# Canleskis/ephemeris-explorer

Hardware: AMD Instinct MI355X
Metric: body-steps/s (higher is better)
Workload: dtype f64

## Files before the change

### ephemeris_explorer_amd/csrc/step_wg.hip

```cpp
#include <algorithm>
#include <type_traits>
#include <utility>

#include "pair_ns.h"

#ifndef EPH_EXPERIMENTS
#define EPH_EXPERIMENTS 0
#endif
#if !EPH_EXPERIMENTS || !defined(EPH_WG_SIDE)
#undef EPH_WG_SIDE
#define EPH_WG_SIDE 0
#endif
#if !EPH_EXPERIMENTS || !defined(EPH_WG_ABLATE)
#undef EPH_WG_ABLATE
#define EPH_WG_ABLATE 0
#endif
#define WG_LOOP_BARRIER() do { if constexpr (!(EPH_WG_ABLATE & 2)) __syncthreads(); } while (0)
#if EPH_EXPERIMENTS && defined(EPH_WG_DIAG_PATCH)
#define EPH_WG_DIAG_PATCH_ON 1
#else
#define EPH_WG_DIAG_PATCH_ON 0
#endif


namespace eph {
namespace EPH_PV_NS {

constexpr int kWgBodies = 16;
constexpr int kDuoThreads = 64 * 6;
constexpr int kDuoTailWave = 5;
constexpr int kWgChainWave = 4;
constexpr int kWgTailWave = 8;
constexpr int kWgThreads = 64 * 12;
constexpr int kWgTileBufs = 6;
constexpr int kWgSplitBufs = 3;

template <int NB>
__device__ __forceinline__ void wg_pair_tile(const double (&xi)[NB], const double (&yi)[NB], const double (&zi)[NB],
                                             const Body4 &pj, bool ieee, double *tile, int b0, int lane) {
    PairPre pre[NB];
    unsigned worst = ieee ? kRangeSpan : mu_key(pj.mu), low = ~0u;
#pragma unroll
    for (int b = 0; b < NB; ++b) {
        pre[b] = pair_pre(xi[b], yi[b], zi[b], pj);
        worst = max(worst, range_key(pre[b].n2));
        low = min(low, pre[b].lo);
    }
    worst = max(worst, low_key(low));
    double c[3 * NB];
    if (__builtin_amdgcn_ballot_w64(worst >= kRangeSpan) == 0) {
#pragma unroll
        for (int b = 0; b < NB; ++b) pair_finish<true>(pre[b], pj.mu, c[3 * b], c[3 * b + 1], c[3 * b + 2]);
    } else {
#pragma unroll
        for (int b = 0; b < NB; ++b) pair_finish<false>(pre[b], pj.mu, c[3 * b], c[3 * b + 1], c[3 * b + 2]);
    }
#pragma unroll
    for (int q = 0; q < 3 * NB; ++q) {
        if constexpr (EPH_WG_ABLATE & 1) asm volatile("" ::"v"(c[q]));
        else tile[(3 * b0 + q) * kRow + lane] = c[q];
    }
}

template <int NB, typename PosPtr>
__device__ __forceinline__ void wg_pair_wave(PosPtr pos, int n, int i0, int b0, double *C, int lane, int tiles, int tdiag, int wbuf) {
    double xi[NB], yi[NB], zi[NB];
#pragma unroll
    for (int b = 0; b < NB; ++b) {
        const int ii = min(i0 + b0 + b, n - 1);
        xi[b] = pos[ii].x;
        yi[b] = pos[ii].y;
        zi[b] = pos[ii].z;
    }
    auto load_src = [&](int t) -> Body4 {
        const int j = min(t, tiles - 1) * kTile + lane;
        return pos[j < n ? j : n - 1];
    };
    Body4 pj = load_src(0);
    Body4 pjn = load_src(1);
    wg_pair_tile<NB>(xi, yi, zi, pj, tdiag == 0, C, b0, lane);
    pj = pjn;
    pjn = load_src(2);
    if (tiles > 1) wg_pair_tile<NB>(xi, yi, zi, pj, tdiag == 1, C + wbuf, b0, lane);
    __syncthreads();
    for (int t = 0; t < tiles; ++t) {
        if (t + 2 < tiles) {
            pj = pjn;
            pjn = load_src(t + 3);
            wg_pair_tile<NB>(xi, yi, zi, pj, tdiag == t + 2, C + ((t + 2) % kWgSplitBufs) * wbuf, b0, lane);
        }
        __syncthreads();
    }
}

template <int NB>
__device__ __forceinline__ void wg_pair_tile2(const double (&xi)[NB], const double (&yi)[NB], const double (&zi)[NB],
                                              const Body4 &pa, const Body4 &pb, bool ieee, double *tile_a, double *tile_b,
                                              int b0, int lane, int self_a = -64, int self_b = -64) {
    PairPre pre[2 * NB];
    unsigned worst = ieee ? kRangeSpan : max(mu_key(pa.mu), mu_key(pb.mu)), low = ~0u;
#pragma unroll
    for (int b = 0; b < NB; ++b) {
        pre[b] = pair_pre(xi[b], yi[b], zi[b], pa);
        pre[NB + b] = pair_pre(xi[b], yi[b], zi[b], pb);
        if constexpr (EPH_WG_DIAG_PATCH_ON) {
            if (lane == self_a + b) { pre[b].n2 = 1.0; pre[b].lo = 0x3ff00000u; }
            if (lane == self_b + b) { pre[NB + b].n2 = 1.0; pre[NB + b].lo = 0x3ff00000u; }
        }
        worst = max(worst, max(range_key(pre[b].n2), range_key(pre[NB + b].n2)));
        low = min(low, min(pre[b].lo, pre[NB + b].lo));
    }
    worst = max(worst, low_key(low));
    double c[6 * NB];
    if (__builtin_amdgcn_ballot_w64(worst >= kRangeSpan) == 0) {
        if constexpr (kPairStaged) {
            double mus[2 * NB];
#pragma unroll
            for (int b = 0; b < NB; ++b) { mus[b] = pa.mu; mus[NB + b] = pb.mu; }
            pair_finish_staged<2 * NB>(pre, mus, c);
        } else {
#pragma unroll
            for (int b = 0; b < NB; ++b) {
                pair_finish<true>(pre[b], pa.mu, c[3 * b], c[3 * b + 1], c[3 * b + 2]);
                pair_finish<true>(pre[NB + b], pb.mu, c[3 * (NB + b)], c[3 * (NB + b) + 1], c[3 * (NB + b) + 2]);
            }
        }
    } else {
#pragma unroll
        for (int b = 0; b < NB; ++b) {
            pair_finish<false>(pre[b], pa.mu, c[3 * b], c[3 * b + 1], c[3 * b + 2]);
            pair_finish<false>(pre[NB + b], pb.mu, c[3 * (NB + b)], c[3 * (NB + b) + 1], c[3 * (NB + b) + 2]);
        }
    }
#pragma unroll
    for (int q = 0; q < 3 * NB; ++q) {
        if constexpr (EPH_WG_ABLATE & 1) {
            asm volatile("" ::"v"(c[q]), "v"(c[3 * NB + q]));
        } else {
            tile_a[(3 * b0 + q) * kRow + lane] = c[q];
            tile_b[(3 * b0 + q) * kRow + lane] = c[3 * NB + q];
        }
    }
}

__device__ __forceinline__ int big_start(int K) { return K < 2 ? K : 2 * K - 2; }
__device__ __forceinline__ int big_count(int tiles) { return tiles <= 2 ? tiles : 2 + (tiles - 2 + 1) / 2; }
template <int NB, typename PosPtr>
__device__ __forceinline__ void wg_pair_wave_big(PosPtr pos, int n, int i0, int b0, double *C, int lane, int tiles, int tdiag, int wbuf) {
    double xi[NB], yi[NB], zi[NB];
#pragma unroll
    for (int b = 0; b < NB; ++b) {
        const int ii = min(i0 + b0 + b, n - 1);
        xi[b] = pos[ii].x;
        yi[b] = pos[ii].y;
        zi[b] = pos[ii].z;
    }
    auto load_src = [&](int t) -> Body4 {
        const int j = min(t, tiles - 1) * kTile + lane;
        return pos[j < n ? j : n - 1];
    };
    auto produce = [&](int K, const Body4 &pa, const Body4 &pb) {
        const int t = big_start(K);
        if (t >= tiles || EPH_WG_SIDE == 2) return;
        double *ta = C + (t % kWgTileBufs) * wbuf, *tb = C + ((t + 1) % kWgTileBufs) * wbuf;
        if constexpr (EPH_WG_DIAG_PATCH_ON) {
            if (K >= 2 && t + 1 < tiles) {
                const int own = i0 + b0;
                wg_pair_tile2<NB>(xi, yi, zi, pa, pb, false, ta, tb, b0, lane, tdiag == t ? own - t * kTile : -64,
                                  tdiag == t + 1 ? own - (t + 1) * kTile : -64);
                return;
            }
        }
        if (K >= 2 && t + 1 < tiles) wg_pair_tile2<NB>(xi, yi, zi, pa, pb, tdiag == t || tdiag == t + 1, ta, tb, b0, lane);
        else wg_pair_tile<NB>(xi, yi, zi, pa, tdiag == t, ta, b0, lane);
    };
    const int TB = big_count(tiles);
    Body4 pa = load_src(0), pb = load_src(1), na = load_src(2), nb = load_src(3);
    produce(0, pa, pa);
    produce(1, pb, pb);
    __syncthreads();
    for (int K = 0; K < TB; ++K) {
        pa = na; pb = nb;
        na = load_src(big_start(K + 3)); nb = load_src(big_start(K + 3) + 1);
        produce(K + 2, pa, pb);
        WG_LOOP_BARRIER();
    }
}
__device__ __forceinline__ void wg_idle_wave(int tiles) {
    __syncthreads();
    for (int T = 0; T < big_count(tiles); ++T) WG_LOOP_BARRIER();
}

__device__ __forceinline__ int phase_start(int P) { return P < 2 ? P : 3 * P - 4; }
__device__ __forceinline__ int phase_count(int tiles) { return tiles <= 2 ? tiles : 2 + (tiles - 2 + 2) / 3; }
__device__ __forceinline__ int phase_tiles(int P, int tiles) { return P < 2 ? 1 : min(3, tiles - phase_start(P)); }

template <int MA, int MB>
__device__ __forceinline__ void pair_finish_staged_split(const PairPre (&pre)[MA + MB], const double (&mu)[MA + MB], double (&c)[3 * (MA + MB)]) {
    PairPre pa[MA], pb[MB];
    double ma[MA], mb[MB], ca[3 * MA], cb[3 * MB];
#pragma unroll
    for (int k = 0; k < MA; ++k) { pa[k] = pre[k]; ma[k] = mu[k]; }
#pragma unroll
    for (int k = 0; k < MB; ++k) { pb[k] = pre[MA + k]; mb[k] = mu[MA + k]; }
    pair_finish_staged<MA>(pa, ma, ca);
    pair_finish_staged<MB>(pb, mb, cb);
#pragma unroll
    for (int k = 0; k < 3 * MA; ++k) c[k] = ca[k];
#pragma unroll
    for (int k = 0; k < 3 * MB; ++k) c[3 * MA + k] = cb[k];
}

template <int NB, int NT, int BS = 1>
__device__ __forceinline__ void wg_pair_block(const double (&xi)[NB], const double (&yi)[NB], const double (&zi)[NB],
                                              const Body4 (&pj)[NT], bool ieee, double *const (&tile)[NT], int b0, int lane,
                                              const int (&self)[NT]) {
    constexpr int M = NB * NT;
    PairPre pre[M];
    double mus[M];
    unsigned worst = ieee ? kRangeSpan : 0u, low = ~0u;
#pragma unroll
    for (int s = 0; s < NT; ++s) {
        worst = max(worst, mu_key(pj[s].mu));
#pragma unroll
        for (int b = 0; b < NB; ++b) {
            const int k = s * NB + b;
            pre[k] = pair_pre(xi[b], yi[b], zi[b], pj[s]);
            mus[k] = pj[s].mu;
            if constexpr (EPH_WG_DIAG_PATCH_ON) {
                if (lane == self[s] + BS * b) { pre[k].n2 = 1.0; pre[k].lo = 0x3ff00000u; }
            }
            worst = max(worst, range_key(pre[k].n2));
            low = min(low, pre[k].lo);
        }
    }
    worst = max(worst, low_key(low));
    double c[3 * M];
    if (__builtin_amdgcn_ballot_w64(worst >= kRangeSpan) == 0) {
        if constexpr (kPairStaged && M == 5 && (kPairVariant == 4 || kPairVariant == 6)) {
            pair_finish_staged_split<3, 2>(pre, mus, c);
        } else if constexpr (kPairStaged) {
            pair_finish_staged<M>(pre, mus, c);
        } else {
#pragma unroll
            for (int k = 0; k < M; ++k) pair_finish<true>(pre[k], mus[k], c[3 * k], c[3 * k + 1], c[3 * k + 2]);
        }
    } else {
#pragma unroll
        for (int k = 0; k < M; ++k) pair_finish<false>(pre[k], mus[k], c[3 * k], c[3 * k + 1], c[3 * k + 2]);
    }
#pragma unroll
    for (int s = 0; s < NT; ++s) {
#pragma unroll
        for (int q = 0; q < 3 * NB; ++q) {
            if constexpr (EPH_WG_ABLATE & 1) asm volatile("" ::"v"(c[3 * NB * s + q]));
            else tile[s][(3 * (b0 + BS * (q / 3)) + q % 3) * kRow + lane] = c[3 * NB * s + q];
        }
    }
}

template <int NB, int BS = 1, typename PosPtr>
__device__ __forceinline__ void wg_pair_wave_deal(PosPtr pos, int n, int i0, int b0, int rank, double *C, int lane, int tiles, int tdiag, int wbuf) {
    double xi[NB], yi[NB], zi[NB];
#pragma unroll
    for (int b = 0; b < NB; ++b) {
        const int ii = min(i0 + b0 + BS * b, n - 1);
        xi[b] = pos[ii].x;
        yi[b] = pos[ii].y;
        zi[b] = pos[ii].z;
    }
    auto load_src = [&](int t) -> Body4 {
        const int j = min(t, tiles - 1) * kTile + lane;
        return pos[j < n ? j : n - 1];
    };
    auto tile_of = [&](int P) { return P < 2 ? (rank == 0 ? P : tiles) : phase_start(P) + rank; };
    auto produce = [&](int t, const Body4 &pj) {
        if (t >= tiles || EPH_WG_SIDE == 2 || (EPH_WG_SIDE == 3 && BS == 1)) return;
        const Body4 src[1] = {pj};
        double *const dst[1] = {C + (t % kWgTileBufs) * wbuf};
        const int self[1] = {EPH_WG_DIAG_PATCH_ON && t == tdiag ? i0 + b0 - t * kTile : -64};
        wg_pair_block<NB, 1, BS>(xi, yi, zi, src, !EPH_WG_DIAG_PATCH_ON && t == tdiag, dst, b0, lane, self);
    };
    const int NP = phase_count(tiles);
    Body4 pj = load_src(tile_of(0)), pjn = load_src(tile_of(1));
    produce(tile_of(0), pj);
    __syncthreads();
    for (int P = 1; P < NP; ++P) {
        pj = pjn;
        pjn = load_src(tile_of(P + 1));
        produce(tile_of(P), pj);
        WG_LOOP_BARRIER();
    }
}
constexpr int kWgShedFirst = 5, kWgShedStride = 5, kWgShedBodies = 3;
template <typename PosPtr>
__device__ __forceinline__ void wg_tail_wave_phases(PosPtr pos, int n, int i0, double *C, int lane, int tiles, int tdiag, int wbuf) {
    wg_pair_wave_deal<kWgShedBodies, kWgShedStride>(pos, n, i0, kWgShedFirst, 2, C, lane, tiles, tdiag, wbuf);
}
template <typename PosPtr>
__device__ __forceinline__ void wg_pair_wave_solo(PosPtr pos, int n, int i0, double *C, int lane, int tiles, int tdiag, int wbuf) {
    const int ii = min(i0, n - 1);
    const double xi[1] = {pos[ii].x}, yi[1] = {pos[ii].y}, zi[1] = {pos[ii].z};
    auto load_src = [&](int t) -> Body4 {
        const int j = min(t, tiles - 1) * kTile + lane;
        return pos[j < n ? j : n - 1];
    };
    auto load_phase = [&](int P, Body4 (&s)[3]) {
        const int t = phase_start(P);
        s[0] = load_src(t);
        if (P >= 2) { s[1] = load_src(t + 1); s[2] = load_src(t + 2); }
    };
    const int NP = phase_count(tiles);
    auto produce = [&](int P, const Body4 (&s)[3]) {
        if (P >= NP || EPH_WG_SIDE == 2) return;
        const int t = phase_start(P), cnt = phase_tiles(P, tiles);
        if (cnt == 3) {
            double *const dst[3] = {C + (t % kWgTileBufs) * wbuf, C + ((t + 1) % kWgTileBufs) * wbuf, C + ((t + 2) % kWgTileBufs) * wbuf};
            const bool own = tdiag >= t && tdiag < t + 3;
            int self[3];
#pragma unroll
            for (int k = 0; k < 3; ++k) self[k] = EPH_WG_DIAG_PATCH_ON && tdiag == t + k ? i0 - (t + k) * kTile : -64;
            wg_pair_block<1, 3>(xi, yi, zi, s, !EPH_WG_DIAG_PATCH_ON && own, dst, 0, lane, self);
        } else {
            auto one = [&](int k, const Body4 &pj) {
                const Body4 src[1] = {pj};
                double *const dst[1] = {C + ((t + k) % kWgTileBufs) * wbuf};
                const int self[1] = {EPH_WG_DIAG_PATCH_ON && tdiag == t + k ? i0 - (t + k) * kTile : -64};
                wg_pair_block<1, 1>(xi, yi, zi, src, !EPH_WG_DIAG_PATCH_ON && tdiag == t + k, dst, 0, lane, self);
            };
            one(0, s[0]);
            if (cnt > 1) one(1, s[1]);
        }
    };
    Body4 s[3], sn[3];
    load_phase(0, s);
    load_phase(1, sn);
    produce(0, s);
    __syncthreads();
    for (int P = 1; P < NP; ++P) {
#pragma unroll
        for (int k = 0; k < 3; ++k) s[k] = sn[k];
        load_phase(P + 1, sn);
        produce(P, s);
        WG_LOOP_BARRIER();
    }
}

__device__ __forceinline__ double chain_full_q(const double *row, double2 (&q)[4][8], double acc) {
    load_chunk(row, 2, q[2]);
    acc = add_chunk(q[0], acc);
    load_chunk(row, 3, q[3]);
    acc = add_chunk(q[1], acc);
    acc = add_chunk(q[2], acc);
    return add_chunk(q[3], acc);
}
__device__ __forceinline__ double chain_full_pf(const double *row, const double *row_next, double2 (&q)[4][8],
                                                double acc) {
    load_chunk(row, 2, q[2]);
    acc = add_chunk(q[0], acc);
    load_chunk(row, 3, q[3]);
    acc = add_chunk(q[1], acc);
    load_chunk(row_next, 0, q[0]);
    acc = add_chunk(q[2], acc);
    load_chunk(row_next, 1, q[1]);
    return add_chunk(q[3], acc);
}

#ifndef EPH_WG_TILE_SPLIT
#define EPH_WG_TILE_SPLIT 2
#endif
constexpr bool wg_tile_split(int wb) { return EPH_WG_TILE_SPLIT == 1 ? wb < 16 : (EPH_WG_TILE_SPLIT == 2 && wb == 4); }
constexpr int wg_split_wave_b(int wb) { return wb == 8 ? 11 : 6; }
template <int WB>
__device__ __forceinline__ int wg_small_body(int wave) {
    if constexpr (WB == 8) {
        switch (wave) { case 1: return 0; case 2: return 1; case 3: return 2; case 5: return 3; case 6: return 4; case 7: return 5;
                        case 9: return 6; case 10: return 7; default: return -1; }
    } else {
        switch (wave) { case 1: return 0; case 2: return 1; case 3: return 2; case 5: return 3; default: return -1; }
    }
}
template <int WB, typename PosPtr>
__device__ __forceinline__ double wg_force_split(PosPtr pos, int n, int i0, double init, double *C, int tid) {
    constexpr int kRows = 3 * WB, kBuf = kRows * kRow;
    const int lane = tid & 63, wave = tid >> 6;
    const int tiles = (n + kTile - 1) / kTile;
    const int tdiag = i0 / kTile;
    double *H = C + kWgSplitBufs * kBuf;
    const int body = wg_small_body<WB>(wave);
    if (body >= 0) { wg_pair_wave<1>(pos, n, i0, body, C, lane, tiles, tdiag, kBuf); return 0.0; }
    const bool isA = wave == kWgChainWave, isB = wave == wg_split_wave_b(WB);
    if (!isA && !isB) { for (int t = 0; t <= tiles; ++t) __syncthreads(); return 0.0; }
    const int ch = lane < kRows ? lane : kRows - 1;
    const double *row = C + ch * kRow;
    const int gself = (i0 % kTile) / WB;
    const int li = (i0 % kTile) + ch / 3;
    double acc = init, accL = 0.0;
    double2 q[4][8];
    auto plain = [&](int t) { return t < tiles && t != tdiag && min(kTile, n - t * kTile) == kTile; };
    auto preload = [&](int t) {
        const double *r = row + (t % kWgSplitBufs) * kBuf;
        load_chunk(r, 0, q[0]); load_chunk(r, 1, q[1]); load_chunk(r, 2, q[2]); load_chunk(r, 3, q[3]);
    };
    __syncthreads();
    if (isA && plain(0)) preload(0);
    for (int t = 0; t < tiles; ++t) {
        const bool mine = ((t & 1) != 0) == isB;
        if (mine) {
            if (t > 0) { acc = H[lane]; accL = H[64 + lane]; }
            if (plain(t)) {
                acc = add_chunk(q[0], acc); acc = add_chunk(q[1], acc); acc = add_chunk(q[2], acc); acc = add_chunk(q[3], acc);
            } else {
                chain_masked<WB>(row + (t % kWgSplitBufs) * kBuf, min(kTile, n - t * kTile), t == tdiag ? gself : -1, li, acc, accL);
            }
            H[lane] = acc;
            H[64 + lane] = accL;
        } else if (plain(t + 1)) {
            preload(t + 1);
        }
        __syncthreads();
    }
    return isA ? H[64 + lane] + H[lane] : 0.0;
}

template <int WB = kWgBodies, bool DUO = false, typename PosPtr>
__device__ __forceinline__ double wg_force(PosPtr pos, int n, int i0, double init, double *C, int tid) {
    constexpr int kRows = 3 * WB, kBuf = kRows * kRow;
    const int lane = tid & 63, wave = tid >> 6;
    const int tiles = (n + kTile - 1) / kTile;
    const int tdiag = i0 / kTile;
    if constexpr (DUO) {
        static_assert(WB == 8, "the duo form is the 8-body workgroup with two bodies per pair wave");
        const int w = __builtin_amdgcn_readfirstlane(wave);
        if (w < 4) { wg_pair_wave_big<2>(pos, n, i0, 2 * w, C, lane, tiles, tdiag, kBuf); return 0.0; }
        if (w == kDuoTailWave) { wg_idle_wave(tiles); return 0.0; }
    } else
    if constexpr (wg_tile_split(WB)) return wg_force_split<WB>(pos, n, i0, init, C, tid);
    else if constexpr (WB != kWgBodies) {
        const int body = wg_small_body<WB>(wave);
        if (body >= 0) { wg_pair_wave_big<1>(pos, n, i0, body, C, lane, tiles, tdiag, kBuf); return 0.0; }
        if (wave != kWgChainWave) { wg_idle_wave(tiles); return 0.0; }
    } else {
        const int w = __builtin_amdgcn_readfirstlane(wave);
        if (w == 0) { wg_pair_wave_solo(pos, n, i0, C, lane, tiles, tdiag, kBuf); return 0.0; }
        if ((w & 3) && w < 8) { wg_pair_wave_deal<5>(pos, n, i0, 5 * (w & 3) - 4, w >> 2, C, lane, tiles, tdiag, kBuf); return 0.0; }
        if (w & 3) { wg_pair_wave_deal<4>(pos, n, i0, 5 * (w & 3) - 4, 2, C, lane, tiles, tdiag, kBuf); return 0.0; }
        if (w == kWgTailWave) { wg_tail_wave_phases(pos, n, i0, C, lane, tiles, tdiag, kBuf); return 0.0; }
    }
    const int ch = lane < kRows ? lane : kRows - 1;
    const double *row = C + ch * kRow;
    const int gself = (i0 % kTile) / WB;
    const int li = (i0 % kTile) + ch / 3;
    double acc = init, accL = 0.0;
    double2 q[4][8];
    if constexpr (WB == kWgBodies || DUO) __builtin_amdgcn_s_setprio(3);
    if constexpr (WB == kWgBodies && !DUO) {
        const int NP = phase_count(tiles);
        __syncthreads();
        for (int P = 0; P < NP; ++P) {
            const int t0 = phase_start(P), nt = phase_tiles(P, tiles);
            const bool whole = nt == 3 && (tdiag < t0 || tdiag > t0 + 2) && n - (t0 + 2) * kTile >= kTile;
            if constexpr (EPH_WG_SIDE == 1) {
            } else if (whole) {
                const double *r0 = row + (t0 % kWgTileBufs) * kBuf, *r1 = row + ((t0 + 1) % kWgTileBufs) * kBuf;
                const double *r2 = row + ((t0 + 2) % kWgTileBufs) * kBuf;
                load_chunk(r0, 0, q[0]);
                load_chunk(r0, 1, q[1]);
                acc = chain_full_pf(r0, r1, q, acc);
                acc = chain_full_pf(r1, r2, q, acc);
                acc = chain_full_q(r2, q, acc);
            } else {
                for (int t = t0; t < t0 + nt; ++t) {
                    const double *r = row + (t % kWgTileBufs) * kBuf;
                    const int cnt = min(kTile, n - t * kTile);
                    if (t != tdiag && cnt == kTile) { acc = chain_full(r, acc); continue; }
                    int lit = li;
                    asm volatile("" : "+v"(lit));
                    chain_masked<WB>(r, cnt, t == tdiag ? gself : -1, lit, acc, accL);
                }
            }
            if (P + 1 < NP) WG_LOOP_BARRIER();
        }
        return accL + acc;
    }
    const int TB = big_count(tiles);
    __syncthreads();
    load_chunk(row, 0, q[0]);
    load_chunk(row, 1, q[1]);
    for (int T = 0; T < TB; ++T) {
#pragma unroll
        for (int hf = 0; hf < 2; ++hf) {
            const int t = big_start(T) + hf;
            if (t >= tiles || (T < 2 && hf)) break;
            const double *r = row + (t % kWgTileBufs) * kBuf;
            const double *rn = row + ((t + 1) % kWgTileBufs) * kBuf;
            const int cnt = min(kTile, n - t * kTile);
            if constexpr (EPH_WG_SIDE == 1) {
            } else if (t != tdiag && cnt == kTile) {
                acc = chain_full_pf(r, rn, q, acc);
            } else {
                chain_masked<WB>(r, cnt, t == tdiag ? gself : -1, li, acc, accL);
                load_chunk(rn, 0, q[0]);
                load_chunk(rn, 1, q[1]);
            }
        }
        WG_LOOP_BARRIER();
    }
    return accL + acc;
}
constexpr int wg_lds_doubles(int wb, bool duo = false) { return (wg_tile_split(wb) && !duo ? kWgSplitBufs * 3 * wb * kRow + 128 : kWgTileBufs * 3 * wb * kRow); }

template <int WB = kWgBodies>
__global__ void __launch_bounds__(kWgThreads) k_accel_wg(int n, int npad, const Body4 *__restrict__ pos,
                                                         const double *__restrict__ acc_init, double *__restrict__ acc_out,
                                                         int lo, int hi, KickDrift kd) {
    __shared__ __attribute__((aligned(16))) double C[wg_lds_doubles(WB)];
    const int tid = threadIdx.x, lane = tid & 63;
    const int i0 = lo + blockIdx.x * WB;
    const int my_i = i0 + lane / 3, cc = lane % 3;
    const bool owner = (tid >> 6) == kWgChainWave && lane < 3 * WB && my_i < hi;
    const double init = (owner && acc_init) ? acc_init[cc * npad + my_i] : 0.0;
    const double a = wg_force<WB>(pos, n, i0, init, C, tid);
    if (owner) {
        acc_out[cc * npad + my_i] = a;
        if (kd.v) kick_drift_one(kd, (size_t)cc * npad + my_i, my_i, cc, a);
    }
}

template <int L, int WB = kWgBodies, bool DUO = false>
__global__ void __launch_bounds__(DUO ? kDuoThreads : kWgThreads) __attribute__((amdgpu_waves_per_eu(3, 3)))
k_lm_step_wg(const LmArgs a) {
    constexpr int kRows = 3 * WB;
    __shared__ __attribute__((aligned(16))) double C[wg_lds_doubles(WB, DUO)];
    const int tid = threadIdx.x, lane = tid & 63;
    const bool chain_wave = (tid >> 6) == kWgChainWave;
    const bool tail_wave = __builtin_amdgcn_readfirstlane(tid >> 6) == (DUO ? kDuoTailWave : kWgTailWave);
    const int i0 = a.lo + blockIdx.x * WB;
    const int cb = lane / 3, cc = lane % 3;
    const int my_i = i0 + cb;
    const bool owner = tail_wave && lane < kRows && my_i < a.hi;
    const size_t lvl = (size_t)3 * a.npad;
    const size_t off = (size_t)cc * a.npad + (owner ? my_i : 0);
    if (tail_wave) {
        double yv[L], av[L];
#pragma unroll
        for (int j = 0; j < L; ++j) {
            const int slot = (a.cur + j) % L;
            yv[j] = a.Y[slot * lvl + off];
            av[j] = j > 0 ? a.A[slot * lvl + off] : 0.0;
        }
        const int tiles = (a.n + kTile - 1) / kTile;
        if constexpr (wg_tile_split(WB) && !DUO) {
            for (int t = 0; t <= tiles; ++t) __syncthreads();
        } else if constexpr (WB == kWgBodies && !DUO) {
            wg_tail_wave_phases(a.pos_cur, a.n, i0, C, lane, tiles, i0 / kTile, 3 * WB * kRow);
        } else {
            wg_idle_wave(tiles);
        }
        __syncthreads();
        if (owner) {
            const double anew = C[lane];
            a.A[(size_t)a.cur * lvl + off] = anew;
            {
                double prev[L];
#pragma unroll
                for (int j = 0; j < L - 1; ++j) prev[j] = av[j + 1];
                prev[L - 1] = 0.0;
                a.V[off] = lm_cowell<L>(anew, prev, yv[0], yv[1], a.cw, a.h, a.hc);
            }
            maybe_sample(a.samp, my_i, cc, a.step, yv[0]);
            if (a.do_predict) {
                av[0] = anew;
                const double ynext = lm_predict<L>(yv, av, a.wa, a.wb, a.hh);
                const int nslot = (a.cur + L - 1) % L;
                a.Y[(size_t)nslot * lvl + off] = ynext;
                reinterpret_cast<double *>(a.pos_next + my_i)[cc] = ynext;
            }
        }
    } else {
        const double anew = wg_force<WB, DUO>(a.pos_cur, a.n, i0, 0.0, C, tid);
        if (chain_wave && lane < kRows) C[lane] = anew;
        __syncthreads();
    }
}

int accel_wg(hipStream_t s, int wb, int n, int npad, const Body4 *pos, const double *acc_init, double *acc_out, int lo, int hi,
             const KickDrift &kd) {
    const dim3 grid((hi - lo + wb - 1) / wb), block(kWgThreads);
    if (wb == 8) hipLaunchKernelGGL(k_accel_wg<8>, grid, block, 0, s, n, npad, pos, acc_init, acc_out, lo, hi, kd);
    else if (wb == 4) hipLaunchKernelGGL(k_accel_wg<4>, grid, block, 0, s, n, npad, pos, acc_init, acc_out, lo, hi, kd);
    else hipLaunchKernelGGL(k_accel_wg<16>, grid, block, 0, s, n, npad, pos, acc_init, acc_out, lo, hi, kd);
    return launched("k_accel_wg");
}
int lm_step_wg(hipStream_t s, int wb, const LmArgs &a) {
    if (wb == 9) {
        const dim3 grid((a.hi - a.lo + 7) / 8), block(kDuoThreads);
        if (a.L == 12) hipLaunchKernelGGL((k_lm_step_wg<12, 8, true>), grid, block, 0, s, a);
        else if (a.L == 13) hipLaunchKernelGGL((k_lm_step_wg<13, 8, true>), grid, block, 0, s, a);
        else return EPH_ERR_UNSUPPORTED;
        return launched("k_lm_step_wg (six waves)");
    }
    const dim3 grid((a.hi - a.lo + wb - 1) / wb), block(kWgThreads);
    if (a.L == 12 && wb == 8) hipLaunchKernelGGL((k_lm_step_wg<12, 8>), grid, block, 0, s, a);
    else if (a.L == 13 && wb == 8) hipLaunchKernelGGL((k_lm_step_wg<13, 8>), grid, block, 0, s, a);
    else if (a.L == 12 && wb == 4) hipLaunchKernelGGL((k_lm_step_wg<12, 4>), grid, block, 0, s, a);
    else if (a.L == 13 && wb == 4) hipLaunchKernelGGL((k_lm_step_wg<13, 4>), grid, block, 0, s, a);
    else if (a.L == 12) hipLaunchKernelGGL((k_lm_step_wg<12, 16>), grid, block, 0, s, a);
    else if (a.L == 13) hipLaunchKernelGGL((k_lm_step_wg<13, 16>), grid, block, 0, s, a);
    else return EPH_ERR_UNSUPPORTED;
    return launched("k_lm_step_wg");
}

}
}
```

Measured before the change: 130.5 million.

## Defer third-tile LDS writes by one interval to overlap with next pair compute

Producer waves that handle the third tile of each three-tile phase now hold that tile's results in registers and write them to shared memory during the next interval, interleaved with the next pair computation. The chain consumer's phase schedule is shifted to match, so a tile's third slice is consumed one barrier interval later, with an extra interval added for some tile counts. The aim is to take LDS store latency off the critical path before each barrier and balance work across intervals. In exchange it raises register pressure, adds a trailing interval, and depends on the six-buffer ring so a held tile never overwrites a slot still being read.

```diff
diff --git a/ephemeris_explorer_amd/csrc/step_wg.hip b/ephemeris_explorer_amd/csrc/step_wg.hip
--- a/ephemeris_explorer_amd/csrc/step_wg.hip
+++ b/ephemeris_explorer_amd/csrc/step_wg.hip
@@ -16,6 +16,10 @@
 #define EPH_WG_ABLATE 0
 #endif
 #define WG_LOOP_BARRIER() do { if constexpr (!(EPH_WG_ABLATE & 2)) __syncthreads(); } while (0)
+#if !EPH_EXPERIMENTS || !defined(EPH_WG_LATE_AT)
+#undef EPH_WG_LATE_AT
+#define EPH_WG_LATE_AT 0
+#endif
 #if EPH_EXPERIMENTS && defined(EPH_WG_DIAG_PATCH)
 #define EPH_WG_DIAG_PATCH_ON 1
 #else
@@ -191,12 +195,18 @@
     for (int T = 0; T < big_count(tiles); ++T) WG_LOOP_BARRIER();
 }
 
+constexpr bool kWgLateThird = kPairVariant == 0 || kPairVariant == 4 || kPairVariant == 5;
+static_assert(kWgTileBufs == 6, "the late third tile needs tile t + 6 to be written two intervals after tile t was read");
 __device__ __forceinline__ int phase_start(int P) { return P < 2 ? P : 3 * P - 4; }
 __device__ __forceinline__ int phase_count(int tiles) { return tiles <= 2 ? tiles : 2 + (tiles - 2 + 2) / 3; }
 __device__ __forceinline__ int phase_tiles(int P, int tiles) { return P < 2 ? 1 : min(3, tiles - phase_start(P)); }
-
-template <int MA, int MB>
-__device__ __forceinline__ void pair_finish_staged_split(const PairPre (&pre)[MA + MB], const double (&mu)[MA + MB], double (&c)[3 * (MA + MB)]) {
+__device__ __forceinline__ int interval_count(int tiles) { return phase_count(tiles) + (kWgLateThird && tiles >= 5 && (tiles - 2) % 3 == 0); }
+__device__ __forceinline__ int chain_first(int I) { return kWgLateThird ? (I <= 2 ? I : 3 * I - 5) : phase_start(I); }
+
+struct NoHook { __device__ __forceinline__ void operator()() const {} };
+template <int MA, int MB, typename Between = NoHook>
+__device__ __forceinline__ void pair_finish_staged_split(const PairPre (&pre)[MA + MB], const double (&mu)[MA + MB], double (&c)[3 * (MA + MB)],
+                                                         Between between = Between()) {
     PairPre pa[MA], pb[MB];
     double ma[MA], mb[MB], ca[3 * MA], cb[3 * MB];
 #pragma unroll
@@ -204,6 +214,7 @@
 #pragma unroll
     for (int k = 0; k < MB; ++k) { pb[k] = pre[MA + k]; mb[k] = mu[MA + k]; }
     pair_finish_staged<MA>(pa, ma, ca);
+    between();
     pair_finish_staged<MB>(pb, mb, cb);
 #pragma unroll
     for (int k = 0; k < 3 * MA; ++k) c[k] = ca[k];
@@ -211,11 +222,19 @@
     for (int k = 0; k < 3 * MB; ++k) c[3 * MA + k] = cb[k];
 }
 
-template <int NB, int NT, int BS = 1>
+template <int NB, int NT, int BS = 1, bool LATE = false>
 __device__ __forceinline__ void wg_pair_block(const double (&xi)[NB], const double (&yi)[NB], const double (&zi)[NB],
                                               const Body4 (&pj)[NT], bool ieee, double *const (&tile)[NT], int b0, int lane,
-                                              const int (&self)[NT]) {
+                                              const int (&self)[NT], double (&held)[3 * NB], double *held_tile) {
     constexpr int M = NB * NT;
+    auto write_held = [&]() {
+#pragma unroll
+        for (int q = 0; q < 3 * NB; ++q) {
+            if constexpr (EPH_WG_ABLATE & 1) asm volatile("" ::"v"(held[q]));
+            else held_tile[(3 * (b0 + BS * (q / 3)) + q % 3) * kRow + lane] = held[q];
+        }
+    };
+    if constexpr (LATE && EPH_WG_LATE_AT == 0) write_held();
     PairPre pre[M];
     double mus[M];
     unsigned worst = ieee ? kRangeSpan : 0u, low = ~0u;
@@ -236,8 +255,12 @@
     }
     worst = max(worst, low_key(low));
     double c[3 * M];
+    constexpr bool kLateMid = LATE && kPairStaged && EPH_WG_LATE_AT == 2 && M >= 2;
     if (__builtin_amdgcn_ballot_w64(worst >= kRangeSpan) == 0) {
-        if constexpr (kPairStaged && M == 5 && (kPairVariant == 4 || kPairVariant == 6)) {
+        if constexpr (LATE && (EPH_WG_LATE_AT == 1 || (EPH_WG_LATE_AT == 2 && !kLateMid))) write_held();
+        if constexpr (kLateMid) {
+            pair_finish_staged_split<M - M / 2, M / 2>(pre, mus, c, write_held);
+        } else if constexpr (kPairStaged && M == 5 && (kPairVariant == 4 || kPairVariant == 6)) {
             pair_finish_staged_split<3, 2>(pre, mus, c);
         } else if constexpr (kPairStaged) {
             pair_finish_staged<M>(pre, mus, c);
@@ -246,17 +269,30 @@
             for (int k = 0; k < M; ++k) pair_finish<true>(pre[k], mus[k], c[3 * k], c[3 * k + 1], c[3 * k + 2]);
         }
     } else {
+        if constexpr (LATE && (EPH_WG_LATE_AT == 1 || EPH_WG_LATE_AT == 2)) write_held();
 #pragma unroll
         for (int k = 0; k < M; ++k) pair_finish<false>(pre[k], mus[k], c[3 * k], c[3 * k + 1], c[3 * k + 2]);
     }
-#pragma unroll
-    for (int s = 0; s < NT; ++s) {
+    if constexpr (LATE && EPH_WG_LATE_AT == 3) write_held();
+#pragma unroll
+    for (int s = 0; s < NT - LATE; ++s) {
 #pragma unroll
         for (int q = 0; q < 3 * NB; ++q) {
             if constexpr (EPH_WG_ABLATE & 1) asm volatile("" ::"v"(c[3 * NB * s + q]));
             else tile[s][(3 * (b0 + BS * (q / 3)) + q % 3) * kRow + lane] = c[3 * NB * s + q];
         }
     }
+    if constexpr (LATE) {
+#pragma unroll
+        for (int q = 0; q < 3 * NB; ++q) held[q] = c[3 * NB * (NT - 1) + q];
+    }
+}
+template <int NB, int NT, int BS = 1>
+__device__ __forceinline__ void wg_pair_block(const double (&xi)[NB], const double (&yi)[NB], const double (&zi)[NB],
+                                              const Body4 (&pj)[NT], bool ieee, double *const (&tile)[NT], int b0, int lane,
+                                              const int (&self)[NT]) {
+    double none[3 * NB];
+    wg_pair_block<NB, NT, BS, false>(xi, yi, zi, pj, ieee, tile, b0, lane, self, none, nullptr);
 }
 
 template <int NB, int BS = 1, typename PosPtr>
@@ -274,22 +310,59 @@
         return pos[j < n ? j : n - 1];
     };
     auto tile_of = [&](int P) { return P < 2 ? (rank == 0 ? P : tiles) : phase_start(P) + rank; };
-    auto produce = [&](int t, const Body4 &pj) {
-        if (t >= tiles || EPH_WG_SIDE == 2 || (EPH_WG_SIDE == 3 && BS == 1)) return;
-        const Body4 src[1] = {pj};
-        double *const dst[1] = {C + (t % kWgTileBufs) * wbuf};
-        const int self[1] = {EPH_WG_DIAG_PATCH_ON && t == tdiag ? i0 + b0 - t * kTile : -64};
-        wg_pair_block<NB, 1, BS>(xi, yi, zi, src, !EPH_WG_DIAG_PATCH_ON && t == tdiag, dst, b0, lane, self);
-    };
-    const int NP = phase_count(tiles);
-    Body4 pj = load_src(tile_of(0)), pjn = load_src(tile_of(1));
-    produce(tile_of(0), pj);
-    __syncthreads();
-    for (int P = 1; P < NP; ++P) {
-        pj = pjn;
-        pjn = load_src(tile_of(P + 1));
-        produce(tile_of(P), pj);
-        WG_LOOP_BARRIER();
+    constexpr bool kOff = EPH_WG_SIDE == 2 || (EPH_WG_SIDE == 3 && BS == 1);
+    const int NI = interval_count(tiles);
+    [[maybe_unused]] const int NP = kWgLateThird ? phase_count(tiles) : NI;
+    if constexpr (NB == 5 || !kWgLateThird) {
+        auto produce = [&](int t, const Body4 &pj) {
+            if (t >= tiles || kOff) return;
+            const Body4 src[1] = {pj};
+            double *const dst[1] = {C + (t % kWgTileBufs) * wbuf};
+            const int self[1] = {EPH_WG_DIAG_PATCH_ON && t == tdiag ? i0 + b0 - t * kTile : -64};
+            wg_pair_block<NB, 1, BS>(xi, yi, zi, src, !EPH_WG_DIAG_PATCH_ON && t == tdiag, dst, b0, lane, self);
+        };
+        Body4 pj = load_src(tile_of(0)), pjn = load_src(tile_of(1));
+        produce(tile_of(0), pj);
+        __syncthreads();
+        for (int P = 1; P < NP; ++P) {
+            pj = pjn;
+            pjn = load_src(tile_of(P + 1));
+            produce(tile_of(P), pj);
+            WG_LOOP_BARRIER();
+        }
+        if (NI > NP) WG_LOOP_BARRIER();
+    } else {
+        static_assert(NB < 5, "the late loop is the rank-2 waves' (four bodies) and wave 8's (three)");
+        double held[3 * NB];
+#pragma unroll
+        for (int q = 0; q < 3 * NB; ++q) held[q] = 0.0;
+        int tprev = tile_of(2);
+        Body4 pj, pjn = load_src(tile_of(2));
+        __syncthreads();
+        for (int I = 1; I < NI; ++I) {
+            const int t = I < 2 ? tiles : tile_of(I);
+            if (I >= 2) {
+                pj = pjn;
+                pjn = load_src(tile_of(I + 1));
+            }
+            double *const late = C + (tprev % kWgTileBufs) * wbuf;
+            if (kOff) {
+            } else if (t < tiles) {
+                const Body4 src[1] = {pj};
+                double *const dst[1] = {nullptr};
+                const int self[1] = {EPH_WG_DIAG_PATCH_ON && t == tdiag ? i0 + b0 - t * kTile : -64};
+                wg_pair_block<NB, 1, BS, true>(xi, yi, zi, src, !EPH_WG_DIAG_PATCH_ON && t == tdiag, dst, b0, lane, self, held, late);
+                tprev = t;
+            } else if (tprev < tiles && I > 2) {
+#pragma unroll
+                for (int q = 0; q < 3 * NB; ++q) {
+                    if constexpr (EPH_WG_ABLATE & 1) asm volatile("" ::"v"(held[q]));
+                    else late[(3 * (b0 + BS * (q / 3)) + q % 3) * kRow + lane] = held[q];
+                }
+                tprev = tiles;
+            }
+            WG_LOOP_BARRIER();
+        }
     }
 }
 constexpr int kWgShedFirst = 5, kWgShedStride = 5, kWgShedBodies = 3;
@@ -310,18 +383,35 @@
         s[0] = load_src(t);
         if (P >= 2) { s[1] = load_src(t + 1); s[2] = load_src(t + 2); }
     };
-    const int NP = phase_count(tiles);
+    const int NI = interval_count(tiles), NP = kWgLateThird ? phase_count(tiles) : NI;
+    double held[3] = {0.0, 0.0, 0.0};
+    int tprev = tiles;
+    auto write_held = [&]() {
+        if (tprev >= tiles) return;
+        double *const late = C + (tprev % kWgTileBufs) * wbuf;
+#pragma unroll
+        for (int q = 0; q < 3; ++q) {
+            if constexpr (EPH_WG_ABLATE & 1) asm volatile("" ::"v"(held[q]));
+            else late[q * kRow + lane] = held[q];
+        }
+        tprev = tiles;
+    };
     auto produce = [&](int P, const Body4 (&s)[3]) {
-        if (P >= NP || EPH_WG_SIDE == 2) return;
+        if (EPH_WG_SIDE == 2) return;
+        if (P >= NP) { write_held(); return; }
         const int t = phase_start(P), cnt = phase_tiles(P, tiles);
         if (cnt == 3) {
-            double *const dst[3] = {C + (t % kWgTileBufs) * wbuf, C + ((t + 1) % kWgTileBufs) * wbuf, C + ((t + 2) % kWgTileBufs) * wbuf};
+            double *const dst[3] = {C + (t % kWgTileBufs) * wbuf, C + ((t + 1) % kWgTileBufs) * wbuf,
+                                    kWgLateThird ? nullptr : C + ((t + 2) % kWgTileBufs) * wbuf};
             const bool own = tdiag >= t && tdiag < t + 3;
             int self[3];
 #pragma unroll
             for (int k = 0; k < 3; ++k) self[k] = EPH_WG_DIAG_PATCH_ON && tdiag == t + k ? i0 - (t + k) * kTile : -64;
-            wg_pair_block<1, 3>(xi, yi, zi, s, !EPH_WG_DIAG_PATCH_ON && own, dst, 0, lane, self);
+            double *const late = C + ((tprev < tiles ? tprev : t + 2) % kWgTileBufs) * wbuf;
+            wg_pair_block<1, 3, 1, kWgLateThird>(xi, yi, zi, s, !EPH_WG_DIAG_PATCH_ON && own, dst, 0, lane, self, held, late);
+            if constexpr (kWgLateThird) tprev = t + 2;
         } else {
+            write_held();
             auto one = [&](int k, const Body4 &pj) {
                 const Body4 src[1] = {pj};
                 double *const dst[1] = {C + ((t + k) % kWgTileBufs) * wbuf};
@@ -337,7 +427,7 @@
     load_phase(1, sn);
     produce(0, s);
     __syncthreads();
-    for (int P = 1; P < NP; ++P) {
+    for (int P = 1; P < NI; ++P) {
 #pragma unroll
         for (int k = 0; k < 3; ++k) s[k] = sn[k];
         load_phase(P + 1, sn);
@@ -455,10 +545,10 @@
     double2 q[4][8];
     if constexpr (WB == kWgBodies || DUO) __builtin_amdgcn_s_setprio(3);
     if constexpr (WB == kWgBodies && !DUO) {
-        const int NP = phase_count(tiles);
+        const int NP = interval_count(tiles);
         __syncthreads();
         for (int P = 0; P < NP; ++P) {
-            const int t0 = phase_start(P), nt = phase_tiles(P, tiles);
+            const int t0 = chain_first(P), nt = min(chain_first(P + 1), tiles) - t0;
             const bool whole = nt == 3 && (tdiag < t0 || tdiag > t0 + 2) && n - (t0 + 2) * kTile >= kTile;
             if constexpr (EPH_WG_SIDE == 1) {
             } else if (whole) {
```

After: 135.3 million, median of 6. 1.04x the previous value.
